# TensorSpeech/TensorFlowASR

Hardware: AMD Instinct MI355X
Metric: audio-hours/sec (train step) Conformer-M RNN-T (higher is better)
Workload: dtype bf16; 1 GPU; Conformer-M transducer full train step (fwd+RNN-T loss+bwd+Adam), LibriSpeech-shaped 16 kHz utterances, 32/GPU, padding=batch, SpecAugment on, dropout 0.1; global_batch=32, parallelism=dp1, params=32461288

## Files before the change

### include/tfasr_hip.h

```cpp
#ifndef TFASR_HIP_H_
#define TFASR_HIP_H_

#include <stddef.h>
#include <stdint.h>

#ifdef __cplusplus
extern "C" {
#endif

#define TFASR_ABI_VERSION 44

typedef enum {
  TFASR_STATUS_SUCCESS = 0,
  TFASR_STATUS_INVALID_VALUE = 1,
  TFASR_STATUS_EXECUTION_FAILED = 2,
  TFASR_STATUS_UNSUPPORTED = 3
} tfasr_status_t;

typedef enum { TFASR_F32 = 0, TFASR_BF16 = 1 } tfasr_dtype_t;

const char* tfasr_status_string(int status);
int tfasr_abi_version(void);
size_t tfasr_launch_count(void);

// ... 65 lines not shown
                        const float* b2, void* y, void* ln, float* mean, float* rstd, void* z, void* h, long rows, int d, int F,
                        float ln_eps, float res_factor, float drop_p, long drop_seed1, long drop_seed2, int dtype, void* stream);
int tfasr_ffn_fused_fwd2(const void* x, const float* gamma, const float* beta, const void* W1, const float* b1, const void* W2,
                         const float* b2, void* y, void* ln, float* mean, float* rstd, void* z, int z_factor, void* h, long rows, int d, int F,
                         float ln_eps, float res_factor, float drop_p, long drop_seed1, long drop_seed2, int dtype, void* stream);
int tfasr_ln_dense_fwd(const void* x, const float* gamma, const float* beta, const void* W, const float* b, void* out, void* ln, float* mean,
                       float* rstd, long rows, int d, int N, float ln_eps, int dtype, void* stream);
int tfasr_layernorm_bwd(const void* dy, const void* x, const float* gamma, const float* mean, const float* rstd,
                        const void* add, void* dx, float* dgamma, float* dbeta, long rows, int C, int dtype,
                        void* stream);
int tfasr_layernorm_bwd_drop(const void* dy, const void* x, const float* gamma, const float* mean, const float* rstd,
                             const void* add, void* dx, float* dgamma, float* dbeta, void* dx_dropped, float drop_p,
                             long drop_seed, long rows, int C, int dtype, void* stream);
int tfasr_layernorm_bwd_part_blocks(long rows, int C, int dtype);
int tfasr_layernorm_bwd_part(const void* dy, const void* x, const float* gamma, const float* mean, const float* rstd, const void* add,
                             void* dx, float* part, void* dx_dropped, float drop_p, long drop_seed, long rows, int C, int dtype,
                             void* stream);
int tfasr_layernorm_bwd_part_n(const void* dy, const void* x, const float* gamma, const float* mean, const float* rstd, const void* add,
                               void* dx, float* part, int nblk, void* dx_dropped, float drop_p, long drop_seed, long rows, int C, int dtype,
                               void* stream);
int tfasr_dense_ln_bwd(const void* dy, const void* W, int K, const void* x, const float* gamma, const float* mean, const float* rstd,
                       const void* add, void* dx, float* part, int nblk, void* dx_dropped, float drop_p, long drop_seed, long rows,
                       int d, float alpha, int dtype, void* stream);
int tfasr_layernorm_bwd_fold(const float* part, int nsets, int nblk, int C, float* const* dgamma, float* const* dbeta, void* stream);
int tfasr_layernorm_bwd_fold_sets(const float* const* part, int nsets, int nblk, int C, float* const* dgamma, float* const* dbeta,
                                  void* stream);
int tfasr_bn_stats(const void* x, float* stats, long rows, int C, int dtype, void* stream);
int tfasr_bn_finalize(const float* stats, float count, const float* gamma, const float* beta, float* fin,
                      float* moving_mean, float* moving_var, float momentum, float eps, int C, int training,
                      void* stream);
int tfasr_bn_finalize_apply_fwd(const void* x, const float* stats, float count, const float* gamma, const float* beta, float* fin,
                                float* moving_mean, float* moving_var, float momentum, float eps, void* y, long rows, int C, int act,
                                int training, int dtype, void* stream);
int tfasr_bn_finalize_apply_fwd_copies(const void* x, const float* stats, int copies, float count, const float* gamma, const float* beta, float* fin,
                                       float* moving_mean, float* moving_var, float momentum, float eps, void* y, long rows, int C, int act,
                                       int training, int dtype, void* stream);
int tfasr_bn_apply_fwd(const void* x, const float* fin, void* y, long rows, int C, int act, int dtype, void* stream);
int tfasr_bn_bwd_stats(const void* x, const void* dy, const float* fin, float* bstats, long rows, int C, int act,
                       int dtype, void* stream);
int tfasr_bn_apply_bwd_grads(const void* x, const void* dy, const float* fin, const float* bstats, float count, void* dx, long rows,
                            int C, int act, float* dgamma, float* dbeta, float grad_scale, int dtype, void* stream);
int tfasr_bn_apply_bwd_grads_copies(const void* x, const void* dy, const float* fin, const float* bstats, int copies, float count, void* dx,
                                    long rows, int C, int act, float* dgamma, float* dbeta, float grad_scale, int dtype, void* stream);
int tfasr_bn_apply_bwd(const void* x, const void* dy, const float* fin, const float* bstats, float count, void* dx,
                       long rows, int C, int act, int dtype, void* stream);

// ... 333 lines not shown
```

### tensorflowasr_amd/csrc/block.hip

```cpp
#include "common.h"
#include <string.h>
#include <stdlib.h>
#include <vector>

extern int g_tfasr_group_beside;

bool tfasr_bn_rows_kernel_ok(int C);
namespace {

struct Arena {
  char* base;
  size_t off, cap;
  bool ok;
  size_t peak;
  void* get(size_t n) {
    const size_t a = (off + 255) & ~(size_t)255;
    if (base && a + n > cap) { ok = false; return nullptr; }
    off = a + n;
    if (off > peak) peak = off;
    return base ? base + a : (void*)(uintptr_t)256;
  }
};

struct Ctx {
// ... 260 lines not shown
      return;
    }
    k->ff_zfactor[m] = 0;
    ln_fwd(x, b0, b0 + 1, k->ff_ln[m], k->ff_mean[m], k->ff_rstd[m]);
    G a; a.act = TFASR_ACT_SWISH; a.prez = k->ff_z[m]; a.drop_p = drop_p(); a.drop_seed = seed(site);
    dense(k->ff_ln[m], b0 + 2, b0 + 3, k->ff_h[m], d, F, a);
    G b; b.res = x; b.beta = c->ffm_res; b.drop_p = drop_p(); b.drop_seed = seed(site + 1);
    b.A = k->ff_h[m]; b.lda = F; b.ta = 0; b.B = wp(b0 + 4); b.ldb = d; b.tb = 0; b.D = y; b.ldd = d; b.M = (int)rows; b.N = d; b.K = F;
    b.bias = fp(b0 + 5);
    gemm(b);
  }
  void ffm_bwd(int m, const void* dy, const void* dy_dropped, void* dx, void* dxd, int site, int next_site) {
    const int b0 = m == 0 ? TFASR_BP_FF1_LN_G : TFASR_BP_FF2_LN_G;
    const int d = c->d, F = c->dff;
    const size_t mark = scratch.off;
    const void* dyd = masked(dy, dy_dropped, rows * d, site + 1);
    void* dz = act(scratch, rows * F);
    {
      G w; w.A = k->ff_h[m]; w.lda = F; w.ta = 1; w.B = dyd; w.ldb = d; w.tb = 0; w.D = gp(b0 + 4); w.ldd = d; w.M = F; w.N = d; w.K = (int)rows;
      w.alpha = c->ffm_res; w.out_f32 = 1; w.accumulate = 1; w.split_k = split_k(F, d, rows);
      w.colsum = gp(b0 + 5);
      w.side = 1;
      gemm(w);
      G g; g.A = dyd; g.lda = d; g.ta = 0; g.B = wp(b0 + 4); g.ldb = d; g.tb = 1; g.D = dz; g.ldd = F; g.M = (int)rows; g.N = F; g.K = d;
      g.alpha = c->ffm_res; g.dact_z = k->ff_z[m];
      if (k->ff_zfactor[m]) g.dact = TFASR_ACT_FACTOR;
      else { g.dact = TFASR_ACT_SWISH; g.drop_p = drop_p(); g.drop_seed = seed(site); }
      gemm(g);
    }
    void* dln = act(scratch, rows * d);
    if (!dense_ln_bwd(dz, k->ff_ln[m], b0 + 2, b0 + 3, F, k->ff_x[m], b0, b0 + 1, k->ff_mean[m], k->ff_rstd[m], dy, dx, dxd, next_site)) {
      dense_bwd(dz, k->ff_ln[m], b0 + 2, b0 + 3, d, F, dln);
      ln_bwd(dln, k->ff_x[m], b0, b0 + 1, k->ff_mean[m], k->ff_rstd[m], dy, dx, dxd, next_site);
    }
    rewind(mark);
  }
  void mhsa_fwd(const void* x, void* y, int site) {
    const int d = c->d, H = c->H, dh = c->dh, HD = H * dh, T = c->T, B = c->B, R1 = 2 * T;
    const float scale = 1.f / sqrtf((float)(c->dh_logical > 0 ? c->dh_logical : dh));
    k->at_x = (void*)x;
    k->at_ln = act(stash, rows * d);
    k->at_mean = f32(stash, rows);
    k->at_rstd = f32(stash, rows);
    k->at_qkv = act(stash, rows * 3 * HD);
    k->at_pext = act(stash, (long)R1 * HD);
    k->at_att = act(stash, rows * HD);
    ln_dense(x, TFASR_BP_AT_LN_G, TFASR_BP_AT_LN_B, k->at_ln, k->at_mean, k->at_rstd, TFASR_BP_AT_QKV_W, TFASR_BP_AT_QKV_B, k->at_qkv, 3 * HD);
    if (!dry && io->pext_pre) {
      k->at_pext = (void*)io->pext_pre;
    } else {
      G p; p.A = P->pe; p.lda = d; p.ta = 0; p.B = wp(TFASR_BP_AT_POS_W); p.ldb = HD; p.tb = 0; p.D = k->at_pext; p.ldd = HD; p.M = R1; p.N = HD; p.K = d;
      p.bias = fp(TFASR_BP_AT_POS_B);
      gemm(p);
    }
    if (k->fused) {
      k->at_lse = f32(stash, (long)B * H * T);
      if (!dry)
        chk(tfasr_relattn_fused_fwd(k->at_qkv, fp(TFASR_BP_AT_U), fp(TFASR_BP_AT_V), k->at_pext, io->lengths, k->at_att, k->at_lse, B, H, T, dh,
// ... 517 lines not shown
```

### tensorflowasr_amd/csrc/gemm_fast.hip

```cpp
#include "common.h"
#include <type_traits>
#include <string.h>
#include <stdlib.h>

typedef __attribute__((ext_vector_type(4))) short short4_t;

#ifdef TFASR_GEMM_TIMING
__device__ long long g_gemm_timing[16 * 32768];
#endif

namespace {

constexpr int BM = 128, BK = 64;
constexpr int A_BYTES = BM * BK * 2;

#define LDS_PTR(p) ((__attribute__((address_space(3))) void*)(p))
#define GLB_PTR(p) ((const __attribute__((address_space(1))) void*)(p))

__device__ __forceinline__ uint32_t lds_u32(const char* s) {
  return (uint32_t)__builtin_amdgcn_readfirstlane((int)(uint32_t)(uintptr_t)s);
}
__device__ __forceinline__ void glds16(const void* g, const char* lds_uniform) {
#ifdef TFASR_GLDS_BUILTIN
  __builtin_amdgcn_global_load_lds(GLB_PTR(g), LDS_PTR(lds_uniform), 16, 0, 0);
// ... 783 lines not shown
  static const int per_cu = 2;
  const int slots = per_cu * num_cus();
  if constexpr (BN_ == 64 && (EPI & (E_WS | E_CSUM | E_LSE)) == 0) {
    static const bool one_off = false;
    static const long one_max = (1L << 30);
    if (!one_off && a.split_k <= 1 && ntiles > slots && ntiles <= one_max * num_cus()) {
      constexpr int SMEM1 = 2 * (A_BYTES + 64 * BK * 2);
      TFASR_KLAUNCH((gemm_fast_one_kernel<TA, TB, EPI>), dim3((unsigned)ntiles), dim3(256), SMEM1, stream, a, (int)tiles.x, (int)tiles.y, (int)tiles.z, (int)ntiles);
      TFASR_CHECK_LAUNCH();
      return TFASR_STATUS_SUCCESS;
    }
  }
  int G = (int)(ntiles < slots ? ntiles : slots);
  if (ntiles >= slots) G &= ~7;
  constexpr int SMEM = 2 * (A_BYTES + BN_ * BK * 2) + 4 * (64 / (BN_ / 16)) * (BN_ / 2 + 4) * 4;
  TFASR_KLAUNCH((gemm_fast_kernel<TA, TB, BN_, EPI>), dim3(G), dim3(256), SMEM, stream, a, (int)tiles.x, (int)tiles.y, (int)tiles.z, (int)ntiles);
  TFASR_CHECK_LAUNCH();
  return TFASR_STATUS_SUCCESS;
}

#include "gemm_big.h"
#include "ffn_fused.h"
#include "dense_ln.h"

template <bool TA, bool TB>
int launch_one(const tfasr_gemm_args& a, hipStream_t stream) {
  const int split = a.split_k > 1 ? a.split_k : 1;
  static const bool bn64_off = false;
  const long t128 = (long)((a.N + 127) / 128) * ((a.M + BM - 1) / BM) * a.nb1 * a.nb2 * split;
  static const long bn64_thr = (1L << 40);
  const long bn64_lim = (split <= 1 && !a.accumulate && !a.colsum && std::min(a.K, a.N) <= 256) ? bn64_thr : std::min(bn64_thr, (long)num_cus());
  const bool narrow = !a.lse_part && !a.seg_a_off && (a.N <= 64 || (!bn64_off && t128 <= bn64_lim && a.N > 64 && !(a.accumulate && a.ws)));
  const int bn = narrow ? 64 : 128;
  dim3 grid((a.N + bn - 1) / bn, (a.M + BM - 1) / BM, a.nb1 * a.nb2 * split);
  if ((long)grid.x * grid.y * grid.z > 0x7fffffffL) return TFASR_STATUS_INVALID_VALUE;
  int need = 0;
  bool generic = false;
  if (!a.accumulate) {
    if (a.out_f32) generic = true;
    if (a.act != TFASR_ACT_NONE || a.prez) { if (a.act == TFASR_ACT_SWISH) need |= E_ACT; else generic = true; }
    if (a.dact_z) { if (a.dact == TFASR_ACT_SWISH) need |= E_DACT; else if (a.dact == TFASR_ACT_FACTOR) need |= E_MUL; else generic = true; }
    if (a.drop_p > 0.f) need |= E_DROP;
    if (a.res) need |= E_RES;
  }
  if (a.bns_out) {
    if constexpr (!TA && TB) {
// ... 236 lines not shown
  a.rows = rows; a.F = N; a.eps = ln_eps;
  const int st = launch_ffn_fused_fwd(a, (hipStream_t)stream);
  TFASR_CHECK_LAUNCH();
  return st;
}

extern "C" int tfasr_dense_ln_bwd(const void* dy, const void* W, int K, const void* x, const float* gamma, const float* mean, const float* rstd,
                                  const void* add, void* dx, float* part, int nblk, void* dx_dropped, float drop_p, long drop_seed, long rows,
                                  int d, float alpha, int dtype, void* stream) {
  if (!dy || !W || !x || !gamma || !mean || !rstd || !dx || !part || rows <= 0 || d <= 0 || K <= 0 || nblk <= 0) return TFASR_STATUS_INVALID_VALUE;
  if (dx_dropped && !(drop_p >= 0.f && drop_p < 1.f)) return TFASR_STATUS_INVALID_VALUE;
  if (dtype != TFASR_BF16 || d != DLN_D || (K % 64) != 0 || rows * (long)d >= (1L << 32)) return TFASR_STATUS_UNSUPPORTED;
  const uintptr_t al = (uintptr_t)dy | (uintptr_t)W | (uintptr_t)x | (uintptr_t)add | (uintptr_t)dx | (uintptr_t)dx_dropped | (uintptr_t)gamma;
  if (al & 15) return TFASR_STATUS_UNSUPPORTED;
  DenseLnArgs a;
  a.dy = (const bf16_t*)dy; a.ldy = K; a.W = (const bf16_t*)W; a.ldw = K; a.K = K; a.x = (const bf16_t*)x; a.gamma = gamma; a.mean = mean; a.rstd = rstd;
  a.add = (const bf16_t*)add; a.dx = (bf16_t*)dx; a.dxd = (bf16_t*)dx_dropped; a.drop_p = dx_dropped ? drop_p : 0.f; a.drop_seed = (uint64_t)drop_seed;
  a.part = part; a.rows = rows; a.alpha = alpha; a.ntiles = 0;
  const int st = launch_dense_ln_bwd(a, nblk, (hipStream_t)stream);
  if (st != TFASR_STATUS_SUCCESS) return st;
  TFASR_CHECK_LAUNCH();
  return TFASR_STATUS_SUCCESS;
}
```

### tensorflowasr_amd/csrc/norm.hip

```cpp
#include "common.h"
#include <stdlib.h>
#include <algorithm>

namespace {

constexpr int MAXC_PER_LANE = 16;

template <typename T>
__global__ __launch_bounds__(256) void ln_fwd_kernel(const T* __restrict__ x, const float* __restrict__ gamma,
                                                     const float* __restrict__ beta, T* __restrict__ y,
                                                     float* __restrict__ mean_out, float* __restrict__ rstd_out,
                                                     long rows, int C, float eps) {
  const int lane = threadIdx.x & 63;
  const long w0 = (long)blockIdx.x * (blockDim.x >> 6) + (threadIdx.x >> 6);
  const long nw = (long)gridDim.x * (blockDim.x >> 6);
  for (long r = w0; r < rows; r += nw) {
    const T* xr = x + r * C;
    float v[MAXC_PER_LANE];
    float s = 0.f;
    int n = 0;
    for (int c = lane; c < C; c += 64, ++n) { v[n] = Num<T>::ld(xr + c); s += v[n]; }
    const float mean = wave_sum(s) / C;
    float q = 0.f;
    for (int i = 0; i < n; ++i) { const float d = v[i] - mean; q += d * d; }
// ... 442 lines not shown
          }
          st8(dxm + base, mv);
        }
      }
    }
  }
#pragma unroll
  for (int k = 0; k < 8; ++k) { red[0][w * RPW + sub][c0 + k] = ag[k]; red[1][w * RPW + sub][c0 + k] = ab[k]; }
  __syncthreads();
  for (int c = threadIdx.x; c < C; c += blockDim.x) {
    float sg = 0.f, sb = 0.f;
    for (int q = 0; q < nw * RPW; ++q) { sg += red[0][q][c]; sb += red[1][q][c]; }
    if (part) {
      part[(long)blockIdx.x * 2 * C + c] = sg;
      part[(long)blockIdx.x * 2 * C + C + c] = sb;
    } else {
      if (dgamma) atomicAdd(dgamma + c, sg);
      if (dbeta) atomicAdd(dbeta + c, sb);
    }
  }
}

constexpr int LNF_MAX = 8;
struct LnFoldArgs { float* dg[LNF_MAX]; float* db[LNF_MAX]; };
__device__ __forceinline__ void ln_fold_slice(const float* __restrict__ p, int nblk, int C, int col, float* dg, float* db) {
  __shared__ float red[4][64];
  const int grp = threadIdx.x >> 6;
  float s0 = 0.f, s1 = 0.f, s2 = 0.f, s3 = 0.f;
  if (col < 2 * C) {
    const int per = (nblk + 3) / 4, b0 = grp * per, b1 = min(nblk, b0 + per);
    int b = b0;
    for (; b + 4 <= b1; b += 4) {
      s0 += p[(long)b * 2 * C]; s1 += p[(long)(b + 1) * 2 * C]; s2 += p[(long)(b + 2) * 2 * C]; s3 += p[(long)(b + 3) * 2 * C];
    }
    for (; b < b1; ++b) s0 += p[(long)b * 2 * C];
  }
  red[grp][threadIdx.x & 63] = (s0 + s1) + (s2 + s3);
  __syncthreads();
  if (grp == 0 && col < 2 * C) {
    const float v = (red[0][threadIdx.x] + red[1][threadIdx.x]) + (red[2][threadIdx.x] + red[3][threadIdx.x]);
    if (col < C) { if (dg) dg[col] += v; }
    else if (db) db[col - C] += v;
  }
}
__global__ __launch_bounds__(256) void ln_bwd_fold_kernel(const float* __restrict__ part, int nblk, int C, LnFoldArgs a) {
  const int set = blockIdx.y, col = blockIdx.x * 64 + (threadIdx.x & 63);
  ln_fold_slice(part + (long)set * nblk * 2 * C + col, nblk, C, col, a.dg[set], a.db[set]);
}
constexpr int LNF_SETS_MAX = 128;
struct LnFoldSets { const float* part[LNF_SETS_MAX]; float* dg[LNF_SETS_MAX]; float* db[LNF_SETS_MAX]; };
__global__ __launch_bounds__(256) void ln_bwd_fold_sets_kernel(int nblk, int C, LnFoldSets a) {
  const int set = blockIdx.y, col = blockIdx.x * 64 + (threadIdx.x & 63);
  ln_fold_slice(a.part[set] + col, nblk, C, col, a.dg[set], a.db[set]);
}

template <typename T, int MODE, int LPR>
__global__ __launch_bounds__(512) void bn_stats_vec_kernel(const T* __restrict__ x, const T* __restrict__ dy,
                                                            const float* __restrict__ fin, float* __restrict__ stats,
                                                            long rows, int C, int act_kind) {
  constexpr int RPW = 64 / LPR;
  __shared__ float red[2][8 * RPW][LPR * 8];
  const int lane = threadIdx.x & 63, li = lane % LPR, sub = lane / LPR, w = threadIdx.x >> 6, nw = blockDim.x >> 6;
  const int cs = blockIdx.y * (LPR * 8);
  const int c0 = cs + li * 8;
  const bool act = c0 < C;
  float a0[8], a1[8], mean[8], rstd[8], sc[8], sh[8];
#pragma unroll
  for (int k = 0; k < 8; ++k) { a0[k] = 0.f; a1[k] = 0.f; }
  ldf8(fin + c0, mean, MODE == 1 && act);
  ldf8(fin + C + c0, rstd, MODE == 1 && act);
  ldf8(fin + 2 * C + c0, sc, MODE == 1 && act);
  ldf8(fin + 3 * C + c0, sh, MODE == 1 && act);
  const long w0 = ((long)blockIdx.x * nw + w) * RPW + sub;
  const long step = (long)gridDim.x * nw * RPW;
  if (act)
    for (long r0 = w0; r0 < rows; r0 += 2 * step) {
// ... 108 lines not shown
extern "C" int tfasr_layernorm_bwd_part_blocks(long rows, int C, int dtype) {
  if (dtype != TFASR_BF16 || rows <= 0 || C <= 0 || (C % 8) || C > 512) return 0;
  return ln_bwd_vec_grid(rows, C, true);
}
extern "C" int tfasr_layernorm_bwd_part(const void* dy, const void* x, const float* gamma, const float* mean, const float* rstd, const void* add,
                                        void* dx, float* part, void* dx_dropped, float drop_p, long drop_seed, long rows, int C, int dtype,
                                        void* stream_) {
  if (!dy || !x || !gamma || !mean || !rstd || !dx || !part || rows <= 0) return TFASR_STATUS_INVALID_VALUE;
  if (dx_dropped && !(drop_p >= 0.f && drop_p < 1.f)) return TFASR_STATUS_INVALID_VALUE;
  if (dtype != TFASR_BF16 || (C % 8) || C > 512 || C <= 0) return TFASR_STATUS_UNSUPPORTED;
  return ln_bwd_vec_launch(dy, x, gamma, mean, rstd, add, dx, nullptr, nullptr, dx_dropped, drop_p, drop_seed, rows, C, part, (hipStream_t)stream_);
}
extern "C" int tfasr_layernorm_bwd_part_n(const void* dy, const void* x, const float* gamma, const float* mean, const float* rstd, const void* add,
                                          void* dx, float* part, int nblk, void* dx_dropped, float drop_p, long drop_seed, long rows, int C, int dtype,
                                          void* stream_) {
  if (!dy || !x || !gamma || !mean || !rstd || !dx || !part || rows <= 0 || nblk <= 0) return TFASR_STATUS_INVALID_VALUE;
  if (dx_dropped && !(drop_p >= 0.f && drop_p < 1.f)) return TFASR_STATUS_INVALID_VALUE;
  if (dtype != TFASR_BF16 || (C % 8) || C > 512 || C <= 0) return TFASR_STATUS_UNSUPPORTED;
  return ln_bwd_vec_launch(dy, x, gamma, mean, rstd, add, dx, nullptr, nullptr, dx_dropped, drop_p, drop_seed, rows, C, part, (hipStream_t)stream_, nblk);
}
extern "C" int tfasr_layernorm_bwd_fold(const float* part, int nsets, int nblk, int C, float* const* dgamma, float* const* dbeta, void* stream_) {
  if (!part || nsets <= 0 || nsets > LNF_MAX || nblk <= 0 || C <= 0 || !dgamma || !dbeta) return TFASR_STATUS_INVALID_VALUE;
  LnFoldArgs a;
  for (int i = 0; i < LNF_MAX; ++i) { a.dg[i] = i < nsets ? dgamma[i] : nullptr; a.db[i] = i < nsets ? dbeta[i] : nullptr; }
  TFASR_KLAUNCH(ln_bwd_fold_kernel, dim3((2 * C + 63) / 64, nsets), dim3(256), 0, (hipStream_t)stream_, part, nblk, C, a);
  TFASR_CHECK_LAUNCH();
  return TFASR_STATUS_SUCCESS;
}

extern "C" int tfasr_layernorm_bwd_fold_sets(const float* const* part, int nsets, int nblk, int C, float* const* dgamma, float* const* dbeta,
                                             void* stream_) {
  if (!part || nsets <= 0 || nsets > LNF_SETS_MAX || nblk <= 0 || C <= 0 || !dgamma || !dbeta) return TFASR_STATUS_INVALID_VALUE;
  LnFoldSets a;
  for (int i = 0; i < LNF_SETS_MAX; ++i) {
    a.part[i] = i < nsets ? part[i] : nullptr;
    a.dg[i] = i < nsets ? dgamma[i] : nullptr;
    a.db[i] = i < nsets ? dbeta[i] : nullptr;
    if (i < nsets && !part[i]) return TFASR_STATUS_INVALID_VALUE;
  }
  TFASR_KLAUNCH(ln_bwd_fold_sets_kernel, dim3((2 * C + 63) / 64, nsets), dim3(256), 0, (hipStream_t)stream_, nblk, C, a);
  TFASR_CHECK_LAUNCH();
  return TFASR_STATUS_SUCCESS;
}

extern "C" int tfasr_layernorm_bwd_drop(const void* dy, const void* x, const float* gamma, const float* mean, const float* rstd,
                                        const void* add, void* dx, float* dgamma, float* dbeta, void* dx_dropped, float drop_p,
                                        long drop_seed, long rows, int C, int dtype, void* stream_) {
  if (!dy || !x || !gamma || !mean || !rstd || !dx || rows <= 0 || C <= 0 || C > 64 * MAXC_PER_LANE)
    return TFASR_STATUS_INVALID_VALUE;
  if (dx_dropped && !(drop_p >= 0.f && drop_p < 1.f)) return TFASR_STATUS_INVALID_VALUE;
  hipStream_t s = (hipStream_t)stream_;
  if (dtype == TFASR_BF16 && (C % 8) == 0 && C <= 512)
    return ln_bwd_vec_launch(dy, x, gamma, mean, rstd, add, dx, dgamma, dbeta, dx_dropped, drop_p, drop_seed, rows, C, nullptr, s);
  const int grid = (int)std::min<long>((rows + 3) / 4, 256L);
  if (dtype == TFASR_F32)
    TFASR_KLAUNCH(ln_bwd_kernel<float>, dim3(grid), dim3(256), 0, s, (const float*)dy, (const float*)x, gamma, mean,
                       rstd, (const float*)add, (float*)dx, dgamma, dbeta, rows, C);
  else
    TFASR_KLAUNCH(ln_bwd_kernel<bf16_t>, dim3(grid), dim3(256), 0, s, (const bf16_t*)dy, (const bf16_t*)x, gamma,
                       mean, rstd, (const bf16_t*)add, (bf16_t*)dx, dgamma, dbeta, rows, C);
  TFASR_CHECK_LAUNCH();
  if (dx_dropped) return tfasr_dropout(dx, dx_dropped, rows * C, drop_p, drop_seed, dtype, stream_);
  return TFASR_STATUS_SUCCESS;
// ... 145 lines not shown
```

### tensorflowasr_amd/kernels.py

```python
import ctypes
import os

import torch

from . import _lib
from ._lib import ACT_FACTOR, ACT_NONE, ACT_SIGMOID, ACT_SWISH, ACT_TANH, ACT_TANH_OUT, TFASR_BF16, TFASR_F32, GemmArgs, check

_WS_CACHE = {}
_SPLITK_WS = False


def _dt(t):
    if t.dtype == torch.float32:
        return TFASR_F32
    if t.dtype == torch.bfloat16:
        return TFASR_BF16
    raise TypeError(f"unsupported activation dtype {t.dtype}")


def _p(t):
    if t is None:
        return None
    if not t.is_cuda:
        raise _lib.TfasrError("tensorflowasr_amd ops need HIP device tensors (no CPU fallback on the product path)")
# ... 360 lines not shown
    check(_L().tfasr_layernorm_bwd_fold(_p(part), 1, nblk, C, dg, db, _stream()), "layernorm_bwd_fold")
    return dx


def dense_ln_bwd(dy, W, x, gamma, mean, rstd, dgamma, dbeta, add=None, dropped=None, drop_p=0.0, drop_seed=0, alpha=1.0):
    rows, d = x.numel() // x.shape[-1], x.shape[-1]
    K = dy.shape[-1]
    nblk = _L().tfasr_layernorm_bwd_part_blocks(rows, d, _dt(x))
    if nblk <= 0:
        return None
    dx = torch.empty_like(x)
    part = torch.empty(nblk * 2 * d, dtype=torch.float32, device=x.device)
    st = _L().tfasr_dense_ln_bwd(_p(dy), _p(W), K, _p(x), _p(gamma), _p(mean), _p(rstd), _p(add), _p(dx), _p(part), nblk, _p(dropped), float(drop_p),
                                 int(drop_seed), rows, d, float(alpha), _dt(x), _stream())
    if st == _lib.STATUS_UNSUPPORTED:
        return None
    check(st, "dense_ln_bwd")
    dg = (ctypes.c_void_p * 1)(dgamma.data_ptr())
    db = (ctypes.c_void_p * 1)(dbeta.data_ptr())
    check(_L().tfasr_layernorm_bwd_fold(_p(part), 1, nblk, d, dg, db, _stream()), "layernorm_bwd_fold")
    return dx


def bn_stats(x, stats):
    rows, C = x.numel() // x.shape[-1], x.shape[-1]
    check(_L().tfasr_bn_stats(_p(x), _p(stats), rows, C, _dt(x), _stream()), "bn_stats")


def bn_finalize(stats, count, gamma, beta, fin, moving_mean, moving_var, momentum=0.99, eps=1e-3, training=True):
    C = gamma.numel()
    check(_L().tfasr_bn_finalize(_p(stats), float(count), _p(gamma), _p(beta), _p(fin), _p(moving_mean), _p(moving_var), momentum, eps, C, int(training), _stream()), "bn_finalize")


def bn_finalize_apply_fwd(x, stats, count, gamma, beta, fin, moving_mean, moving_var, act=ACT_NONE, y=None, momentum=0.99, eps=1e-3, training=True,
                          copies=1):
    rows, C = x.numel() // x.shape[-1], x.shape[-1]
    if y is None:
        y = torch.empty_like(x)
    st = _L().tfasr_bn_finalize_apply_fwd_copies(_p(x), _p(stats), int(copies), float(count), _p(gamma), _p(beta), _p(fin), _p(moving_mean), _p(moving_var),
                                                 momentum, eps, _p(y), rows, C, act, int(training), _dt(x), _stream())
    if st == _lib.STATUS_UNSUPPORTED:
        return None
    check(st, "bn_finalize_apply_fwd")
    return y


# ... 1073 lines not shown
```

Measured before the change: 4.724 audio-hours/sec.

## Fuse FFN backward dgrad GEMMs with activation-grad and LayerNorm backward in one kernel

Adds a fused kernel for the feed-forward module backward. It computes dy·W2ᵀ, applies the gate factor to form dz (written out for the weight gradient), multiplies by W1ᵀ to get the LN-output gradient, and runs LayerNorm backward with residual add and dropout, all per 64-row tile and kept in LDS/registers. This removes the separate dz GEMM, dense dgrad GEMM and LN backward launches along with the intermediate dln round trip through HBM. The LN-fold path now merges consecutive partial sets that target the same gamma/beta so the extra tile sets fold in one pass. It only applies for bf16, d=256 with the factor activation, and a timing/debug hook is compiled in behind a macro.

```diff
diff --git a/include/tfasr_hip.h b/include/tfasr_hip.h
--- a/include/tfasr_hip.h
+++ b/include/tfasr_hip.h
@@ -111,6 +111,9 @@
 int tfasr_dense_ln_bwd(const void* dy, const void* W, int K, const void* x, const float* gamma, const float* mean, const float* rstd,
                        const void* add, void* dx, float* part, int nblk, void* dx_dropped, float drop_p, long drop_seed, long rows,
                        int d, float alpha, int dtype, void* stream);
+int tfasr_ffn_fused_bwd(const void* dyd, const void* g, const void* W1, const void* W2, int F, const void* x, const float* gamma,
+                        const float* mean, const float* rstd, const void* add, void* dz, void* dx, float* part, int nblk, void* dx_dropped,
+                        float drop_p, long drop_seed, long rows, int d, float alpha, int dtype, void* stream);
 int tfasr_layernorm_bwd_fold(const float* part, int nsets, int nblk, int C, float* const* dgamma, float* const* dbeta, void* stream);
 int tfasr_layernorm_bwd_fold_sets(const float* const* part, int nsets, int nblk, int C, float* const* dgamma, float* const* dbeta,
                                   void* stream);
diff --git a/tensorflowasr_amd/csrc/block.hip b/tensorflowasr_amd/csrc/block.hip
--- a/tensorflowasr_amd/csrc/block.hip
+++ b/tensorflowasr_amd/csrc/block.hip
@@ -306,6 +306,11 @@
       w.colsum = gp(b0 + 5);
       w.side = 1;
       gemm(w);
+      if (ffn_bwd_fused(m, dyd, dz, dy, dx, dxd, next_site)) {
+        dense_bwd(dz, k->ff_ln[m], b0 + 2, b0 + 3, d, F, nullptr);
+        rewind(mark);
+        return;
+      }
       G g; g.A = dyd; g.lda = d; g.ta = 0; g.B = wp(b0 + 4); g.ldb = d; g.tb = 1; g.D = dz; g.ldd = F; g.M = (int)rows; g.N = F; g.K = d;
       g.alpha = c->ffm_res; g.dact_z = k->ff_z[m];
       if (k->ff_zfactor[m]) g.dact = TFASR_ACT_FACTOR;
@@ -318,6 +323,27 @@
       ln_bwd(dln, k->ff_x[m], b0, b0 + 1, k->ff_mean[m], k->ff_rstd[m], dy, dx, dxd, next_site);
     }
     rewind(mark);
+  }
+  bool ffn_bwd_fused(int m, const void* dyd, void* dz, const void* add, void* dx, void* dxd, int next_site) {
+    const int b0 = m == 0 ? TFASR_BP_FF1_LN_G : TFASR_BP_FF2_LN_G;
+    if (dry || !k->ff_zfactor[m] || !k->ff_z[m] || !k->ln_part || k->ln_nblk <= 0 || c->dtype != TFASR_BF16 || c->d != 256 || (c->dff % 64) != 0) return false;
+    const char* sw = getenv("TFASR_FFN_BWD_FUSED");
+    if (sw && sw[0] == '0') return false;
+    const int need = (int)(((rows + 63) / 64 + k->ln_nblk - 1) / k->ln_nblk);
+    if (k->ln_nsets + need > 8) return false;
+    const bool with_drop = dxd && drop_p() > 0.f && next_site >= 0;
+    float* part = k->ln_part + (size_t)k->ln_nsets * k->ln_nblk * 2 * c->d;
+    const int fst = tfasr_ffn_fused_bwd(dyd, k->ff_z[m], wp(b0 + 2), wp(b0 + 4), c->dff, k->ff_x[m], fp(b0), k->ff_mean[m], k->ff_rstd[m], add, dz, dx, part,
+                                        need * k->ln_nblk, with_drop ? dxd : nullptr, with_drop ? drop_p() : 0.f, with_drop ? seed(next_site) : 0, rows,
+                                        c->d, c->ffm_res, c->dtype, s);
+    if (fst == TFASR_STATUS_UNSUPPORTED) return false;
+    chk(fst);
+    for (int q = 0; q < need; ++q) {
+      k->ln_dg[k->ln_nsets] = gp(b0);
+      k->ln_db[k->ln_nsets] = gp(b0 + 1);
+      ++k->ln_nsets;
+    }
+    return true;
   }
   void mhsa_fwd(const void* x, void* y, int site) {
     const int d = c->d, H = c->H, dh = c->dh, HD = H * dh, T = c->T, B = c->B, R1 = 2 * T;
diff --git a/tensorflowasr_amd/csrc/ffn_bwd_fused.h b/tensorflowasr_amd/csrc/ffn_bwd_fused.h
--- /dev/null
+++ b/tensorflowasr_amd/csrc/ffn_bwd_fused.h
@@ -0,0 +1,334 @@
+#pragma once
+
+struct FfnBwdArgs {
+  const bf16_t* dyd; const bf16_t* g; const bf16_t* W1; const bf16_t* W2;
+  const bf16_t* x; const float* gamma; const float* mean; const float* rstd; const bf16_t* add;
+  bf16_t* dz; bf16_t* dx; bf16_t* dxd; float* part;
+  long rows; int F; int ntiles; float alpha, drop_p; uint64_t drop_seed;
+  long long* dbg;
+};
+
+constexpr int FFB_SMEM = 2 * 32768 + 2 * 8192;
+
+__global__ __launch_bounds__(256, 2) void ffn_fused_bwd_kernel(const FfnBwdArgs p) {
+#ifdef TFASR_FFN_TIMING
+  long long ph[8] = {0, 0, 0, 0, 0, 0, 0, 0};
+  long long tp = __builtin_readcyclecounter();
+#endif
+  constexpr int D = 256, BMR = 64, NW = 4, PCS = 8, PG = 2;
+  constexpr int W2_OFF = 0, W1_OFF = 32768, SH_OFF = 65536, SG_OFF = 65536 + 8192;
+  extern __shared__ __attribute__((aligned(16))) char smem[];
+  const int lane = threadIdx.x & 63, w = __builtin_amdgcn_readfirstlane(threadIdx.x >> 6);
+  const int wr = w >> 1, wc = w & 1;
+  const int r = lane & 15, g = lane >> 4;
+  const int tile = blockIdx.x;
+  if (tile >= p.ntiles) {
+    for (int c = threadIdx.x; c < 2 * D; c += 256) p.part[(long)tile * 2 * D + c] = 0.f;
+    return;
+  }
+  const long m0 = (long)tile * BMR;
+  const int F = p.F, NC = F / 64;
+  const int nrow_tile = (int)min((long)BMR, p.rows - m0);
+  const bool counted = nrow_tile == BMR;
+
+  uint32_t off1[PCS], off2[PCS], offg[PG];
+#pragma unroll
+  for (int n = 0; n < PCS; ++n) {
+    const int pid = w + n * NW, pp = lane & 7;
+    { const int s = pid >> 3, nn = (pid & 7) * 8 + (lane >> 3);
+      off2[n] = (uint32_t)((nn * D + s * 64 + ((pp ^ key_d(nn)) << 3)) * 2); }
+    { const int nn = pid * 8 + (lane >> 3);
+      off1[n] = (uint32_t)((nn * F + ((pp ^ key_d(nn)) << 3)) * 2); }
+  }
+#pragma unroll
+  for (int n = 0; n < PG; ++n) {
+    const int row = (w + n * NW) * 8 + (lane >> 3), pp = lane & 7;
+    offg[n] = (uint32_t)((min(row, nrow_tile - 1) * F + ((pp ^ key_d(row)) << 3)) * 2);
+  }
+  auto issue_w2 = [&](int cc) {
+    const char* src = reinterpret_cast<const char*>(p.W2 + (long)min(cc, NC - 1) * 64 * D);
+#pragma unroll
+    for (int n = 0; n < PCS; ++n) glds16_s(src, off2[n], smem + W2_OFF + __builtin_amdgcn_readfirstlane((w + n * NW) * 1024));
+  };
+  auto issue_w1 = [&](int cc) {
+    const char* src = reinterpret_cast<const char*>(p.W1 + min(cc, NC - 1) * 64);
+#pragma unroll
+    for (int n = 0; n < PCS; ++n) glds16_s(src, off1[n], smem + W1_OFF + __builtin_amdgcn_readfirstlane((w + n * NW) * 1024));
+  };
+  auto issue_g = [&](int cc) {
+    const char* src = reinterpret_cast<const char*>(p.g + m0 * F + min(cc, NC - 1) * 64);
+#pragma unroll
+    for (int n = 0; n < PG; ++n) glds16_s(src, offg[n], smem + SG_OFF + __builtin_amdgcn_readfirstlane((w + n * NW) * 1024));
+  };
+
+  {
+    const char* src = reinterpret_cast<const char*>(p.dyd + m0 * D);
+#pragma unroll
+    for (int n = 0; n < PCS; ++n) {
+      const int pid = w + n * NW, s = pid >> 3, row = (pid & 7) * 8 + (lane >> 3), pp = lane & 7;
+      const uint32_t off = (uint32_t)((min(row, nrow_tile - 1) * D + s * 64 + ((pp ^ key_d(row)) << 3)) * 2);
+      glds16_s(src, off, smem + W1_OFF + __builtin_amdgcn_readfirstlane(pid * 1024));
+    }
+  }
+  issue_w2(0);
+  issue_g(0);
+  asm volatile("s_waitcnt vmcnt(%0)" ::"n"(PCS + PG) : "memory");
+  lds_only_barrier();
+  short8_t dyf[2][8];
+#pragma unroll
+  for (int i = 0; i < 2; ++i)
+#pragma unroll
+    for (int ks = 0; ks < 8; ++ks) dyf[i][ks] = frag_direct(smem + W1_OFF + (ks >> 1) * 8192, wr * 32 + i * 16 + r, (ks & 1) * 4 + g);
+  FFN_TICK(0)
+
+  float4_t acc1[2][2], acc2[2][8];
+#pragma unroll
+  for (int i = 0; i < 2; ++i)
+#pragma unroll
+    for (int j = 0; j < 8; ++j) acc2[i][j] = float4_t{0.f, 0.f, 0.f, 0.f};
+
+  auto gemm1 = [&]() {
+#pragma unroll
+    for (int i = 0; i < 2; ++i)
+#pragma unroll
+      for (int j = 0; j < 2; ++j) acc1[i][j] = float4_t{0.f, 0.f, 0.f, 0.f};
+#pragma unroll
+    for (int kp = 0; kp < 4; ++kp) {
+      short8_t bf[2][2];
+#pragma unroll
+      for (int kk = 0; kk < 2; ++kk)
+#pragma unroll
+        for (int j = 0; j < 2; ++j) bf[kk][j] = frag_direct(smem + W2_OFF + kp * 8192, wc * 32 + j * 16 + r, kk * 4 + g);
+#pragma unroll
+      for (int kk = 0; kk < 2; ++kk)
+#pragma unroll
+        for (int i = 0; i < 2; ++i)
+#pragma unroll
+          for (int j = 0; j < 2; ++j) acc1[i][j] = __builtin_amdgcn_mfma_f32_16x16x32_bf16(bf[kk][j], dyf[i][2 * kp + kk], acc1[i][j], 0, 0, 0);
+      __builtin_amdgcn_sched_barrier(0);
+    }
+  };
+  auto zlds = [&]() {
+    const char* sG = smem + SG_OFF;
+    char* sH = smem + SH_OFF;
+#pragma unroll
+    for (int j = 0; j < 2; ++j) {
+      const int k = wc * 32 + j * 16 + g * 4;
+#pragma unroll
+      for (int i = 0; i < 2; ++i) {
+        const int row = wr * 32 + i * 16 + r;
+        const int at = row * 128 + (((k >> 3) ^ key_d(row)) << 4) + (k & 7) * 2;
+        const uint2 gv = *reinterpret_cast<const uint2*>(sG + at);
+        uint2 v;
+        v.x = pack2_bf16((p.alpha * acc1[i][j][0]) * __uint_as_float(gv.x << 16), (p.alpha * acc1[i][j][1]) * __uint_as_float(gv.x & 0xffff0000u));
+        v.y = pack2_bf16((p.alpha * acc1[i][j][2]) * __uint_as_float(gv.y << 16), (p.alpha * acc1[i][j][3]) * __uint_as_float(gv.y & 0xffff0000u));
+        *reinterpret_cast<uint2*>(sH + at) = v;
+      }
+    }
+  };
+  auto rowpass = [&](int cc, auto FAST_) {
+    constexpr bool FAST = decltype(FAST_)::value;
+    bf16_t* zbase = p.dz + m0 * F + cc * 64;
+#pragma unroll
+    for (int ps = 0; ps < 2; ++ps) {
+      const int row = ps * 32 + (threadIdx.x >> 3), pp = threadIdx.x & 7;
+      const uint4 v = *reinterpret_cast<const uint4*>(smem + SH_OFF + row * 128 + ((pp ^ key_d(row)) << 4));
+      if constexpr (FAST) *reinterpret_cast<uint4*>(zbase + (row * F + pp * 8)) = v;
+      else if (row < nrow_tile) *reinterpret_cast<uint4*>(zbase + (row * F + pp * 8)) = v;
+    }
+  };
+  auto gemm2 = [&]() {
+    const char* sH = smem + SH_OFF;
+    const char* sW1 = smem + W1_OFF;
+#pragma unroll
+    for (int kk = 0; kk < 2; ++kk) {
+      short8_t af[2];
+#pragma unroll
+      for (int i = 0; i < 2; ++i) af[i] = frag_direct(sH, wr * 32 + i * 16 + r, kk * 4 + g);
+#pragma unroll
+      for (int jh = 0; jh < 2; ++jh) {
+        short8_t bf[4];
+#pragma unroll
+        for (int j = 0; j < 4; ++j) bf[j] = frag_direct(sW1, wc * 128 + (jh * 4 + j) * 16 + r, kk * 4 + g);
+#pragma unroll
+        for (int i = 0; i < 2; ++i)
+#pragma unroll
+          for (int j = 0; j < 4; ++j) acc2[i][jh * 4 + j] = __builtin_amdgcn_mfma_f32_16x16x32_bf16(bf[j], af[i], acc2[i][jh * 4 + j], 0, 0, 0);
+        __builtin_amdgcn_sched_barrier(0);
+      }
+    }
+  };
+
+  for (int c = 0; c < NC; ++c) {
+    if (counted && c > 0) asm volatile("s_waitcnt vmcnt(%0)" ::"n"(2) : "memory"); else asm volatile("s_waitcnt vmcnt(0)" ::: "memory");
+    lds_only_barrier();
+    issue_w1(c);
+    FFN_TICK(1)
+    gemm1();
+    zlds();
+    FFN_TICK(2)
+    lds_only_barrier();
+    issue_w2(c + 1);
+    issue_g(c + 1);
+    FFN_TICK(1)
+    if (counted) rowpass(c, std::true_type{}); else rowpass(c, std::false_type{});
+    FFN_TICK(3)
+    if (counted) asm volatile("s_waitcnt vmcnt(%0)" ::"n"(PCS + PG + 2) : "memory"); else asm volatile("s_waitcnt vmcnt(0)" ::: "memory");
+    lds_only_barrier();
+    FFN_TICK(1)
+    gemm2();
+    FFN_TICK(4)
+  }
+
+  const bool odd = (g & 1) != 0;
+  float d8[2][4][8];
+#pragma unroll
+  for (int i = 0; i < 2; ++i)
+#pragma unroll
+    for (int jp = 0; jp < 4; ++jp) {
+      float recv[4];
+#pragma unroll
+      for (int e = 0; e < 4; ++e)
+        recv[e] = __uint_as_float(xor16_get(__float_as_uint(odd ? acc2[i][2 * jp][e] : acc2[i][2 * jp + 1][e]), odd));
+#pragma unroll
+      for (int e = 0; e < 4; ++e) {
+        d8[i][jp][e] = odd ? recv[e] : acc2[i][2 * jp][e];
+        d8[i][jp][4 + e] = odd ? acc2[i][2 * jp + 1][e] : recv[e];
+      }
+    }
+  const int cb = wc * 128 + (odd ? 16 : 0) + (g & 2) * 4;
+  uint4 xr[2][4], ar[2][4];
+  float mr[2], rr[2];
+  bool live[2];
+#pragma unroll
+  for (int i = 0; i < 2; ++i) {
+    const long row = m0 + wr * 32 + i * 16 + r;
+    live[i] = row < p.rows;
+    const long rc = live[i] ? row : p.rows - 1;
+    mr[i] = p.mean[rc];
+    rr[i] = p.rstd[rc];
+#pragma unroll
+    for (int jp = 0; jp < 4; ++jp) xr[i][jp] = *reinterpret_cast<const uint4*>(p.x + rc * D + cb + jp * 32);
+  }
+  float gm[4][8];
+#pragma unroll
+  for (int jp = 0; jp < 4; ++jp) ld8(p.gamma + cb + jp * 32, gm[jp]);
+  asm volatile("s_waitcnt vmcnt(0)" ::: "memory");
+  __syncthreads();
+  float* red = reinterpret_cast<float*>(smem + W2_OFF);
+  float* csum = red + 2 * BMR * 2;
+#pragma unroll
+  for (int i = 0; i < 2; ++i) {
+    float s1 = 0.f, s2 = 0.f;
+#pragma unroll
+    for (int jp = 0; jp < 4; ++jp) {
+      float xv[8];
+      unpack8(xr[i][jp], xv);
+#pragma unroll
+      for (int e = 0; e < 8; ++e) {
+        const float d = live[i] ? d8[i][jp][e] : 0.f;
+        d8[i][jp][e] = d;
+        const float xhat = (xv[e] - mr[i]) * rr[i];
+        const float dg = d * gm[jp][e];
+        s1 += dg;
+        s2 += dg * xhat;
+      }
+    }
+    s1 = xor32_sum(xor16_sum(s1));
+    s2 = xor32_sum(xor16_sum(s2));
+    if (g == 0) *reinterpret_cast<float2*>(red + ((wc * BMR + wr * 32 + i * 16 + r) * 2)) = make_float2(s1, s2);
+  }
+#pragma unroll
+  for (int i = 0; i < 2; ++i)
+#pragma unroll
+    for (int jp = 0; jp < 4; ++jp) ar[i][jp] = make_uint4(0u, 0u, 0u, 0u);
+  if (p.add) {
+#pragma unroll
+    for (int i = 0; i < 2; ++i) {
+      const long row = m0 + wr * 32 + i * 16 + r;
+      const long rc = live[i] ? row : p.rows - 1;
+#pragma unroll
+      for (int jp = 0; jp < 4; ++jp) ar[i][jp] = *reinterpret_cast<const uint4*>(p.add + rc * D + cb + jp * 32);
+    }
+  }
+  __syncthreads();
+  const float invC = 1.f / D;
+  const bool drop = p.dxd != nullptr && p.drop_p > 0.f;
+  const float drop_inv = 1.f / (1.f - p.drop_p);
+  const uint32_t dkey = drop_key(p.drop_seed), dthr = drop_thr(p.drop_p);
+  float s1r[2], s2r[2];
+#pragma unroll
+  for (int i = 0; i < 2; ++i) {
+    const int rl = wr * 32 + i * 16 + r;
+    const float2 t0 = *reinterpret_cast<const float2*>(red + rl * 2), t1 = *reinterpret_cast<const float2*>(red + (BMR + rl) * 2);
+    s1r[i] = (t0.x + t1.x) * invC;
+    s2r[i] = (t0.y + t1.y) * invC;
+  }
+#pragma unroll
+  for (int jp = 0; jp < 4; ++jp) {
+    float ag[8], ab[8];
+#pragma unroll
+    for (int e = 0; e < 8; ++e) { ag[e] = 0.f; ab[e] = 0.f; }
+#pragma unroll
+    for (int i = 0; i < 2; ++i) {
+      const long row = m0 + wr * 32 + i * 16 + r;
+      float xv[8], o[8];
+      unpack8(xr[i][jp], xv);
+      unpack8(ar[i][jp], o);
+#pragma unroll
+      for (int e = 0; e < 8; ++e) {
+        const float d = d8[i][jp][e];
+        const float xhat = (xv[e] - mr[i]) * rr[i];
+        ag[e] += d * xhat;
+        ab[e] += d;
+        o[e] += rr[i] * (d * gm[jp][e] - s1r[i] - xhat * s2r[i]);
+      }
+      if (live[i]) {
+        uint4 v;
+        v.x = pack2_bf16(o[0], o[1]); v.y = pack2_bf16(o[2], o[3]); v.z = pack2_bf16(o[4], o[5]); v.w = pack2_bf16(o[6], o[7]);
+        *reinterpret_cast<uint4*>(p.dx + row * D + cb + jp * 32) = v;
+        if (drop) {
+          const uint64_t e0 = (uint64_t)(row * D + cb + jp * 32);
+          const uint32_t vv[4] = {v.x, v.y, v.z, v.w};
+          uint32_t uu[4];
+#pragma unroll
+          for (int q = 0; q < 4; ++q) {
+            const uint32_t hh = drop_mix(dkey, (uint32_t)((e0 + 2 * q) >> 1), (uint32_t)((e0 + 2 * q) >> 33));
+            const float q0 = (hh & 0xffffu) >= dthr ? __uint_as_float(vv[q] << 16) * drop_inv : 0.f;
+            const float q1 = (hh >> 16) >= dthr ? __uint_as_float(vv[q] & 0xffff0000u) * drop_inv : 0.f;
+            uu[q] = pack2_bf16(q0, q1);
+          }
+          *reinterpret_cast<uint4*>(p.dxd + row * D + cb + jp * 32) = make_uint4(uu[0], uu[1], uu[2], uu[3]);
+        }
+      }
+    }
+#pragma unroll
+    for (int e = 0; e < 8; ++e) { ag[e] = row16_sum(ag[e]); ab[e] = row16_sum(ab[e]); }
+    if (r == 0) {
+      st8(csum + (wr * 2 + 0) * D + cb + jp * 32, ag);
+      st8(csum + (wr * 2 + 1) * D + cb + jp * 32, ab);
+    }
+  }
+  __syncthreads();
+  {
+    float* po = p.part + (long)tile * 2 * D;
+    const int t = threadIdx.x;
+    po[t] = csum[t] + csum[2 * D + t];
+    po[D + t] = csum[D + t] + csum[3 * D + t];
+  }
+#ifdef TFASR_FFN_TIMING
+  FFN_TICK(5)
+  if (p.dbg && blockIdx.x == 0 && threadIdx.x == 0)
+    for (int k = 0; k < 8; ++k) p.dbg[k] = ph[k];
+#endif
+}
+
+static int launch_ffn_fused_bwd(FfnBwdArgs a, int nslots, hipStream_t stream) {
+  const long tiles = (a.rows + 63) / 64;
+  if (tiles > nslots) return TFASR_STATUS_UNSUPPORTED;
+  a.ntiles = (int)tiles;
+  static bool attr_done = false;
+  if (!attr_done) { (void)hipFuncSetAttribute((const void*)ffn_fused_bwd_kernel, hipFuncAttributeMaxDynamicSharedMemorySize, FFB_SMEM); attr_done = true; }
+  TFASR_KLAUNCH(ffn_fused_bwd_kernel, dim3((unsigned)nslots), dim3(256), FFB_SMEM, stream, a);
+  return TFASR_STATUS_SUCCESS;
+}
diff --git a/tensorflowasr_amd/csrc/gemm_fast.hip b/tensorflowasr_amd/csrc/gemm_fast.hip
--- a/tensorflowasr_amd/csrc/gemm_fast.hip
+++ b/tensorflowasr_amd/csrc/gemm_fast.hip
@@ -829,6 +829,7 @@
 #include "gemm_big.h"
 #include "ffn_fused.h"
 #include "dense_ln.h"
+#include "ffn_bwd_fused.h"
 
 template <bool TA, bool TB>
 int launch_one(const tfasr_gemm_args& a, hipStream_t stream) {
@@ -1111,3 +1112,36 @@
   TFASR_CHECK_LAUNCH();
   return TFASR_STATUS_SUCCESS;
 }
+
+extern "C" int tfasr_ffn_fused_bwd(const void* dyd, const void* g, const void* W1, const void* W2, int F, const void* x, const float* gamma,
+                                   const float* mean, const float* rstd, const void* add, void* dz, void* dx, float* part, int nblk,
+                                   void* dx_dropped, float drop_p, long drop_seed, long rows, int d, float alpha, int dtype, void* stream) {
+  if (!dyd || !W1 || !W2 || !x || !gamma || !mean || !rstd || !dz || !dx || !part || rows <= 0 || d <= 0 || F <= 0 || nblk <= 0) return TFASR_STATUS_INVALID_VALUE;
+  if (dx_dropped && !(drop_p >= 0.f && drop_p < 1.f)) return TFASR_STATUS_INVALID_VALUE;
+  if (!g || dtype != TFASR_BF16 || d != 256 || (F % 64) != 0 || F > 4096 || rows * (long)F >= (1L << 32)) return TFASR_STATUS_UNSUPPORTED;
+  const uintptr_t al = (uintptr_t)dyd | (uintptr_t)g | (uintptr_t)W1 | (uintptr_t)W2 | (uintptr_t)x | (uintptr_t)add | (uintptr_t)dz | (uintptr_t)dx |
+                       (uintptr_t)dx_dropped | (uintptr_t)gamma | (uintptr_t)part;
+  if (al & 15) return TFASR_STATUS_UNSUPPORTED;
+  FfnBwdArgs a;
+  a.dyd = (const bf16_t*)dyd; a.g = (const bf16_t*)g; a.W1 = (const bf16_t*)W1; a.W2 = (const bf16_t*)W2; a.x = (const bf16_t*)x; a.gamma = gamma;
+  a.mean = mean; a.rstd = rstd; a.add = (const bf16_t*)add; a.dz = (bf16_t*)dz; a.dx = (bf16_t*)dx; a.dxd = (bf16_t*)dx_dropped; a.part = part;
+  a.rows = rows; a.F = F; a.ntiles = 0; a.alpha = alpha; a.drop_p = dx_dropped ? drop_p : 0.f; a.drop_seed = (uint64_t)drop_seed;
+  a.dbg = nullptr;
+#ifdef TFASR_FFN_TIMING
+  static long long* dbg_buf = nullptr;
+  if (!dbg_buf && hipMalloc((void**)&dbg_buf, 64) != hipSuccess) dbg_buf = nullptr;
+  a.dbg = dbg_buf;
+#endif
+  const int st = launch_ffn_fused_bwd(a, nblk, (hipStream_t)stream);
+  if (st != TFASR_STATUS_SUCCESS) return st;
+#ifdef TFASR_FFN_TIMING
+  if (dbg_buf) {
+    long long h[8];
+    if (hipStreamSynchronize((hipStream_t)stream) == hipSuccess && hipMemcpy(h, dbg_buf, 64, hipMemcpyDeviceToHost) == hipSuccess)
+      fprintf(stderr, "[ffn_bwd_timing] prologue %lld | per-kernel sums: wait+barrier+dma-issue %lld gemm1+dz->lds %lld rowpass %lld gemm2 %lld | epilogue %lld\n",
+              h[0], h[1], h[2], h[3], h[4], h[5]);
+  }
+#endif
+  TFASR_CHECK_LAUNCH();
+  return TFASR_STATUS_SUCCESS;
+}
diff --git a/tensorflowasr_amd/csrc/norm.hip b/tensorflowasr_amd/csrc/norm.hip
--- a/tensorflowasr_amd/csrc/norm.hip
+++ b/tensorflowasr_amd/csrc/norm.hip
@@ -488,7 +488,7 @@
 }
 
 constexpr int LNF_MAX = 8;
-struct LnFoldArgs { float* dg[LNF_MAX]; float* db[LNF_MAX]; };
+struct LnFoldArgs { float* dg[LNF_MAX]; float* db[LNF_MAX]; int first[LNF_MAX]; int mult[LNF_MAX]; };
 __device__ __forceinline__ void ln_fold_slice(const float* __restrict__ p, int nblk, int C, int col, float* dg, float* db) {
   __shared__ float red[4][64];
   const int grp = threadIdx.x >> 6;
@@ -511,13 +511,13 @@
 }
 __global__ __launch_bounds__(256) void ln_bwd_fold_kernel(const float* __restrict__ part, int nblk, int C, LnFoldArgs a) {
   const int set = blockIdx.y, col = blockIdx.x * 64 + (threadIdx.x & 63);
-  ln_fold_slice(part + (long)set * nblk * 2 * C + col, nblk, C, col, a.dg[set], a.db[set]);
+  ln_fold_slice(part + (long)a.first[set] * nblk * 2 * C + col, nblk * a.mult[set], C, col, a.dg[set], a.db[set]);
 }
 constexpr int LNF_SETS_MAX = 128;
-struct LnFoldSets { const float* part[LNF_SETS_MAX]; float* dg[LNF_SETS_MAX]; float* db[LNF_SETS_MAX]; };
+struct LnFoldSets { const float* part[LNF_SETS_MAX]; float* dg[LNF_SETS_MAX]; float* db[LNF_SETS_MAX]; unsigned char mult[LNF_SETS_MAX]; };
 __global__ __launch_bounds__(256) void ln_bwd_fold_sets_kernel(int nblk, int C, LnFoldSets a) {
   const int set = blockIdx.y, col = blockIdx.x * 64 + (threadIdx.x & 63);
-  ln_fold_slice(a.part[set] + col, nblk, C, col, a.dg[set], a.db[set]);
+  ln_fold_slice(a.part[set] + col, nblk * a.mult[set], C, col, a.dg[set], a.db[set]);
 }
 
 template <typename T, int MODE, int LPR>
@@ -672,8 +672,14 @@
 extern "C" int tfasr_layernorm_bwd_fold(const float* part, int nsets, int nblk, int C, float* const* dgamma, float* const* dbeta, void* stream_) {
   if (!part || nsets <= 0 || nsets > LNF_MAX || nblk <= 0 || C <= 0 || !dgamma || !dbeta) return TFASR_STATUS_INVALID_VALUE;
   LnFoldArgs a;
-  for (int i = 0; i < LNF_MAX; ++i) { a.dg[i] = i < nsets ? dgamma[i] : nullptr; a.db[i] = i < nsets ? dbeta[i] : nullptr; }
-  TFASR_KLAUNCH(ln_bwd_fold_kernel, dim3((2 * C + 63) / 64, nsets), dim3(256), 0, (hipStream_t)stream_, part, nblk, C, a);
+  int n = 0;
+  for (int i = 0; i < LNF_MAX; ++i) { a.dg[i] = nullptr; a.db[i] = nullptr; a.first[i] = 0; a.mult[i] = 1; }
+  for (int i = 0; i < nsets; ++i) {
+    if (n > 0 && dgamma[i] == a.dg[n - 1] && dbeta[i] == a.db[n - 1]) { ++a.mult[n - 1]; continue; }
+    a.dg[n] = dgamma[i]; a.db[n] = dbeta[i]; a.first[n] = i; a.mult[n] = 1;
+    ++n;
+  }
+  TFASR_KLAUNCH(ln_bwd_fold_kernel, dim3((2 * C + 63) / 64, n), dim3(256), 0, (hipStream_t)stream_, part, nblk, C, a);
   TFASR_CHECK_LAUNCH();
   return TFASR_STATUS_SUCCESS;
 }
@@ -682,13 +688,18 @@
                                              void* stream_) {
   if (!part || nsets <= 0 || nsets > LNF_SETS_MAX || nblk <= 0 || C <= 0 || !dgamma || !dbeta) return TFASR_STATUS_INVALID_VALUE;
   LnFoldSets a;
-  for (int i = 0; i < LNF_SETS_MAX; ++i) {
-    a.part[i] = i < nsets ? part[i] : nullptr;
-    a.dg[i] = i < nsets ? dgamma[i] : nullptr;
-    a.db[i] = i < nsets ? dbeta[i] : nullptr;
-    if (i < nsets && !part[i]) return TFASR_STATUS_INVALID_VALUE;
-  }
-  TFASR_KLAUNCH(ln_bwd_fold_sets_kernel, dim3((2 * C + 63) / 64, nsets), dim3(256), 0, (hipStream_t)stream_, nblk, C, a);
+  int n = 0;
+  for (int i = 0; i < LNF_SETS_MAX; ++i) { a.part[i] = nullptr; a.dg[i] = nullptr; a.db[i] = nullptr; a.mult[i] = 1; }
+  for (int i = 0; i < nsets; ++i) {
+    if (!part[i]) return TFASR_STATUS_INVALID_VALUE;
+    if (n > 0 && dgamma[i] == a.dg[n - 1] && dbeta[i] == a.db[n - 1] && part[i] == a.part[n - 1] + (size_t)a.mult[n - 1] * nblk * 2 * C) {
+      ++a.mult[n - 1];
+      continue;
+    }
+    a.part[n] = part[i]; a.dg[n] = dgamma[i]; a.db[n] = dbeta[i]; a.mult[n] = 1;
+    ++n;
+  }
+  TFASR_KLAUNCH(ln_bwd_fold_sets_kernel, dim3((2 * C + 63) / 64, n), dim3(256), 0, (hipStream_t)stream_, nblk, C, a);
   TFASR_CHECK_LAUNCH();
   return TFASR_STATUS_SUCCESS;
 }
diff --git a/tensorflowasr_amd/kernels.py b/tensorflowasr_amd/kernels.py
--- a/tensorflowasr_amd/kernels.py
+++ b/tensorflowasr_amd/kernels.py
@@ -406,6 +406,29 @@
     return dx
 
 
+def ffn_fused_bwd(dyd, g, W1, W2, x, gamma, mean, rstd, dgamma, dbeta, add=None, dropped=None, drop_p=0.0, drop_seed=0, alpha=1.0):
+    rows, d = x.numel() // x.shape[-1], x.shape[-1]
+    F = W1.shape[-1]
+    nblk = _L().tfasr_layernorm_bwd_part_blocks(rows, d, _dt(x))
+    if nblk <= 0:
+        return None
+    nsets = ((rows + 63) // 64 + nblk - 1) // nblk
+    if nsets > 8:
+        return None
+    dz = torch.empty(rows, F, dtype=x.dtype, device=x.device)
+    dx = torch.empty_like(x)
+    part = torch.empty(nsets * nblk * 2 * d, dtype=torch.float32, device=x.device)
+    st = _L().tfasr_ffn_fused_bwd(_p(dyd), _p(g), _p(W1), _p(W2), F, _p(x), _p(gamma), _p(mean), _p(rstd), _p(add), _p(dz), _p(dx), _p(part),
+                                  nsets * nblk, _p(dropped), float(drop_p), int(drop_seed), rows, d, float(alpha), _dt(x), _stream())
+    if st == _lib.STATUS_UNSUPPORTED:
+        return None
+    check(st, "ffn_fused_bwd")
+    dg = (ctypes.c_void_p * nsets)(*([dgamma.data_ptr()] * nsets))
+    db = (ctypes.c_void_p * nsets)(*([dbeta.data_ptr()] * nsets))
+    check(_L().tfasr_layernorm_bwd_fold(_p(part), nsets, nblk, d, dg, db, _stream()), "layernorm_bwd_fold")
+    return dz, dx
+
+
 def bn_stats(x, stats):
     rows, C = x.numel() // x.shape[-1], x.shape[-1]
     check(_L().tfasr_bn_stats(_p(x), _p(stats), rows, C, _dt(x), _stream()), "bn_stats")
```

New measurement: 4.740 audio-hours/sec, median of 6. No clear change (+0.3%).
